# aleju/cat-generator

Measured on AMD Instinct MI355X. Metric: images/sec per G+D step, G32up-c 32x32 RGB bs=128 per GPU, higher is better.
Workload: dtype f32

## Files before the change

### cat-generator_amd/csrc/gemm.hip

```cpp
#include "common.h"
#include <stdlib.h>
#include <algorithm>
#include <mutex>
#include <type_traits>
#include <unordered_map>
#include <vector>

namespace {

typedef float f32x16 __attribute__((ext_vector_type(16)));
typedef unsigned int u32x4 __attribute__((ext_vector_type(4)));

constexpr int BK = 16;
constexpr unsigned OOB = 0x80000000u;
#ifdef CG_TRACE
__device__ unsigned long long* g_trace;
#define CG_STAMP(slot)                                                                                                  \
    do {                                                                                                                \
        if (threadIdx.x == 0 && g_trace) {                                                                              \
            const long wg = blockIdx.x + (long)gridDim.x * (blockIdx.y + (long)gridDim.y * blockIdx.z);                  \
            g_trace[wg * 8 + (slot)] = wall_clock64();                                                                  \
            if ((slot) == 0) {                                                                                          \
                g_trace[wg * 8 + 4] = __builtin_amdgcn_s_getreg((31 << 11) | 4);                       \
                g_trace[wg * 8 + 5] = __builtin_amdgcn_s_getreg((31 << 11) | 20);                     \
// ... 1614 lines not shown
    const int c = blockIdx.x * 32 + cl;
    float s = 0.f;
    if (c < Cout)
        for (int i = ln; i < S * P; i += 8) s += bp[(long)(i / P) * sstride + (long)(i % P) * Cout + c];
    sh[ln][cl] = s;
    __syncthreads();
    if (ln == 0 && c < Cout) {
        float t = 0.f;
#pragma unroll
        for (int r = 0; r < 8; ++r) t += sh[r][cl];
        gb[c] += scale * t;
    }
}

__global__ __launch_bounds__(256) void pack_weight_kernel(const float* w, float* wf, float* wb, int Cout, int Cin, int KK,
                                                          int wb_map) {
    __shared__ float sh[32][33];
    const int lo = threadIdx.x & 31, hi = threadIdx.x >> 5;
    const int ci0 = blockIdx.x * 32, co0 = blockIdx.y * 32;
    {
        const int tap = blockIdx.z;
#pragma unroll
        for (int j = 0; j < 4; ++j) {
            const int ci = ci0 + lo, co_l = hi + 8 * j, co = co0 + co_l;
            float v = 0.f;
            if (ci < Cin && co < Cout) {
                v = w[((long)co * Cin + ci) * KK + tap];
                if (wb) wb[wb_map ? ((long)co * KK + tap) * Cin + ci : ((long)(KK - 1 - tap) * Cout + co) * Cin + ci] = v;
            }
            sh[lo][co_l] = v;
        }
        if (wf) {
            __syncthreads();
#pragma unroll
            for (int j = 0; j < 4; ++j) {
                const int co = co0 + lo, ci_l = hi + 8 * j, ci = ci0 + ci_l;
                if (ci < Cin && co < Cout) wf[((long)tap * Cin + ci) * Cout + co] = sh[ci_l][lo];
            }
        }
    }
}

constexpr int kPackBatch = 48;
struct PackBatch {
    const float* w[kPackBatch]; float* wf[kPackBatch]; float* wb[kPackBatch];
    int Cout[kPackBatch], Cin[kPackBatch], KK[kPackBatch], first[kPackBatch + 1];
    unsigned long long map_mask;
    int n;
};
__global__ __launch_bounds__(256) void pack_weight_batch_kernel(PackBatch b) {
    __shared__ float sh[32][33];
    int e = 0;
    while (e + 1 < b.n && (int)blockIdx.x >= b.first[e + 1]) ++e;
    const float* w = b.w[e]; float* wf = b.wf[e]; float* wb = b.wb[e];
    const int Cout = b.Cout[e], Cin = b.Cin[e], KK = b.KK[e];
    const bool wb_map = (b.map_mask >> e) & 1ull;
    const int nbx = (Cin + 31) / 32, nby = (Cout + 31) / 32;
    int r = (int)blockIdx.x - b.first[e];
    const int bx = r % nbx; r /= nbx;
    const int by = r % nby;
    const int tap = r / nby;
    const int lo = threadIdx.x & 31, hi = threadIdx.x >> 5;
    const int ci0 = bx * 32, co0 = by * 32;
#pragma unroll
    for (int j = 0; j < 4; ++j) {
        const int ci = ci0 + lo, co_l = hi + 8 * j, co = co0 + co_l;
        float v = 0.f;
        if (ci < Cin && co < Cout) {
            v = w[((long)co * Cin + ci) * KK + tap];
            if (wb) wb[wb_map ? ((long)co * KK + tap) * Cin + ci : ((long)(KK - 1 - tap) * Cout + co) * Cin + ci] = v;
        }
        sh[lo][co_l] = v;
    }
    if (wf) {
        __syncthreads();
#pragma unroll
        for (int j = 0; j < 4; ++j) {
            const int co = co0 + lo, ci_l = hi + 8 * j, ci = ci0 + ci_l;
            if (ci < Cin && co < Cout) wf[((long)tap * Cin + ci) * Cout + co] = sh[ci_l][lo];
        }
    }
}

template <int K>
__global__ __launch_bounds__(256) void pack_weight_ups2_fast_kernel(const float* w, float* wf, float* wb, int Cout, int Cin) {
    constexpr int KK = K * K, PAD = (K - 1) / 2, KPD = K == 3 ? 2 : 3, KP = KPD * KPD;
    __shared__ float sh[KP][32][33];
    const int lo = threadIdx.x & 31, hi = threadIdx.x >> 5;
    const int ci0 = blockIdx.x * 32, co0 = blockIdx.y * 32;
    float v[4][KK];
#pragma unroll
    for (int j = 0; j < 4; ++j) {
        const int ci = ci0 + lo, co = co0 + hi + 8 * j;
        const bool ok = ci < Cin && co < Cout;
        const float* src = w + ((long)co * Cin + ci) * KK;
#pragma unroll
        for (int t = 0; t < KK; ++t) v[j][t] = ok ? src[t] : 0.f;
    }
#pragma unroll
    for (int p = 0; p < 4; ++p) {
#pragma unroll
        for (int j = 0; j < 4; ++j) {
            float acc[KP];
#pragma unroll
            for (int t = 0; t < KP; ++t) acc[t] = 0.f;
#pragma unroll
            for (int dy = 0; dy < K; ++dy)
#pragma unroll
                for (int dx = 0; dx < K; ++dx)
                    acc[phase_map(p >> 1, dy, PAD) * KPD + phase_map(p & 1, dx, PAD)] += v[j][dy * K + dx];
            const int ci = ci0 + lo, co_l = hi + 8 * j, co = co0 + co_l;
#pragma unroll
            for (int t = 0; t < KP; ++t) {
                if (wb && ci < Cin && co < Cout) wb[(((long)p * KP + t) * Cout + co) * Cin + ci] = acc[t];
                sh[t][lo][co_l] = acc[t];
            }
        }
        if (wf) {
            __syncthreads();
#pragma unroll
            for (int t = 0; t < KP; ++t)
#pragma unroll
                for (int j = 0; j < 4; ++j) {
                    const int co = co0 + lo, ci_l = hi + 8 * j, ci = ci0 + ci_l;
                    if (ci < Cin && co < Cout) wf[(((long)p * KP + t) * Cin + ci) * Cout + co] = sh[t][ci_l][lo];
                }
            __syncthreads();
        }
    }
}

__global__ __launch_bounds__(256) void pack_weight_ups2_kernel(const float* w, float* wf, float* wb, int Cout, int Cin, int k,
                                                               int pad, int kp, int CI_T) {
    extern __shared__ float sh[];
    const int KK = k * k, KP = kp * kp;
    const int run = CI_T * KK, ld = run + 1;
    const int ci0 = blockIdx.x * CI_T, co0 = blockIdx.y * 32;
    const int cis = min(CI_T, Cin - ci0);
    for (int idx = threadIdx.x; idx < 32 * run; idx += 256) {
        const int j = idx % run, co_l = idx / run;
        if (co0 + co_l < Cout && j < cis * KK) sh[co_l * ld + j] = w[((long)(co0 + co_l) * Cin + ci0) * KK + j];
    }
    __syncthreads();
    const int n = 4 * KP * CI_T * 32;
    for (int pass = 0; pass < 2; ++pass) {
        if (pass == 0 ? wf == nullptr : wb == nullptr) continue;
        for (int idx = threadIdx.x; idx < n; idx += 256) {
            int co_l, ci_l, q;
            if (pass == 0) { co_l = idx & 31; const int r = idx >> 5; ci_l = r % CI_T; q = r / CI_T; }
            else { ci_l = idx % CI_T; const int r = idx / CI_T; co_l = r & 31; q = r >> 5; }
            if (co0 + co_l >= Cout || ci_l >= cis) continue;
            const int tp = q % KP, p = q / KP;
            const int ry = tp / kp, rx = tp - ry * kp;
            const float* src = sh + co_l * ld + ci_l * KK;
            float s = 0.f;
            for (int dy = 0; dy < k; ++dy) {
                if (phase_map(p >> 1, dy, pad) != ry) continue;
                for (int dx = 0; dx < k; ++dx)
                    if (phase_map(p & 1, dx, pad) == rx) s += src[dy * k + dx];
            }
            if (pass == 0) wf[(((long)p * KP + tp) * Cin + ci0 + ci_l) * Cout + co0 + co_l] = s;
            else wb[(((long)p * KP + tp) * Cout + co0 + co_l) * Cin + ci0 + ci_l] = s;
        }
    }
}

template <int CO, int LP>
__global__ __launch_bounds__(256) void skinny_conv3x3_kernel(const float* __restrict__ x, const float* __restrict__ w,
                                                             const float* __restrict__ bias, float* __restrict__ y, int N,
                                                             int H, int W) {
    constexpr int Cin = 4 * LP;
    const int sub = threadIdx.x & (LP - 1);
    float wr[9][4][CO];
#pragma unroll
    for (int t = 0; t < 9; ++t)
#pragma unroll
        for (int j = 0; j < 4; ++j)
#pragma unroll
            for (int co = 0; co < CO; ++co) wr[t][j][co] = w[((long)t * Cin + sub * 4 + j) * CO + co];
    const long npix = (long)N * H * W;
    const long grp0 = (blockIdx.x * 256L + threadIdx.x) / LP;
    const long ngrp = gridDim.x * 256L / LP;
    const long iters = (npix + ngrp - 1) / ngrp;
    for (long it = 0; it < iters; ++it) {
        const long pix = grp0 + it * ngrp;
        const bool live = pix < npix;
        const unsigned pc = live ? (unsigned)pix : 0u;
        const unsigned row = pc / (unsigned)W;
        const int ox = (int)(pc - row * (unsigned)W), oy = (int)(row % (unsigned)H);
        const long n = row / (unsigned)H;
        float acc[CO];
#pragma unroll
        for (int co = 0; co < CO; ++co) acc[co] = 0.f;
        float4 v[9];
#pragma unroll
        for (int t = 0; t < 9; ++t) {
            const int iy = oy + t / 3 - 1, ix = ox + t % 3 - 1;
            const bool ok = live && iy >= 0 && iy < H && ix >= 0 && ix < W;
            const int cy = min(max(iy, 0), H - 1), cx = min(max(ix, 0), W - 1);
            const float4 q = ld4(x + ((n * H + cy) * (long)W + cx) * Cin + sub * 4);
            v[t] = ok ? q : make_float4(0.f, 0.f, 0.f, 0.f);
        }
#pragma unroll
        for (int t = 0; t < 9; ++t)
#pragma unroll
            for (int co = 0; co < CO; ++co)
                acc[co] += v[t].x * wr[t][0][co] + v[t].y * wr[t][1][co] + v[t].z * wr[t][2][co] + v[t].w * wr[t][3][co];
#pragma unroll
        for (int off = LP >> 1; off > 0; off >>= 1)
#pragma unroll
// ... 820 lines not shown
        CG_LAUNCH_CHECK();
        if (gb && gb[gi]) {
            hipLaunchKernelGGL(bias_part_reduce_kernel, dim3(cg::cdiv(Cout, 32)), dim3(256), 0, st,
                               (const float*)a.bias_part + (long)gi * g.nphase * Cout, gb[gi], p.splits, g.nphase,
                               (long)ZP * Cout, Cout, scale);
            CG_LAUNCH_CHECK();
        }
    }
    return 0;
}

}

int cg_conv2d_wgrad(void* stream, const float* x, const float* dy, float* gw, float* gb, int N, int Hp, int Wp, int Cin,
                    int Cout, int kH, int kW, int padH, int padW, int ups, float scale, void* ws, size_t ws_bytes) {
    CG_REQUIRE(x && dy && gw, "cg_conv2d_wgrad: null pointer");
    return cg_conv2d_wgrad_grouped(stream, 1, &x, &dy, &gw, &gb, N, Hp, Wp, Cin, Cout, kH, kW, padH, padW, ups, scale, ws,
                                   ws_bytes);
}

static int pack_ci_tile(int Cin, int KK) {
    int t = 1;
    while (t * 2 * KK <= 448 && t < Cin) t *= 2;
    return t;
}

int cg_pack_conv_weight(void* stream, const float* w, float* wf, float* wb, int Cout, int Cin, int kH, int kW) {
    CG_REQUIRE(w && (wf || wb), "cg_pack_conv_weight: null pointer");
    CG_REQUIRE(Cout > 0 && Cin > 0 && kH > 0 && kW > 0, "cg_pack_conv_weight: bad dims");
    const int KK = kH * kW;
    hipLaunchKernelGGL(pack_weight_kernel, dim3(cg::cdiv(Cin, 32), cg::cdiv(Cout, 32), KK), dim3(256), 0, cg::S(stream), w,
                       wf, wb, Cout, Cin, KK, 0);
    CG_LAUNCH_CHECK();
    return cg::wino3_note_pack(cg::S(stream), 1, &w, &wf, &wb, &Cout, &Cin, &kH, &kW, nullptr);
}

int cg_pack_conv_weight_map(void* stream, const float* w, float* wf, float* wbT, int Cout, int Cin, int kH, int kW) {
    CG_REQUIRE(w && (wf || wbT), "cg_pack_conv_weight_map: null pointer");
    CG_REQUIRE(Cout > 0 && Cin > 0 && kH > 0 && kW > 0, "cg_pack_conv_weight_map: bad dims");
    const int KK = kH * kW;
    hipLaunchKernelGGL(pack_weight_kernel, dim3(cg::cdiv(Cin, 32), cg::cdiv(Cout, 32), KK), dim3(256), 0, cg::S(stream), w,
                       wf, wbT, Cout, Cin, KK, 1);
    CG_LAUNCH_CHECK();
    return 0;
}

int cg_pack_conv_weight_batch(void* stream, int n, const float* const* w_canonical, float* const* wf, float* const* wb,
                              const int* Cout, const int* Cin, const int* kH, const int* kW, const int* wb_map) {
    CG_REQUIRE(n >= 0 && w_canonical && wf && wb && Cout && Cin && kH && kW, "cg_pack_conv_weight_batch: null pointer");
    for (int i0 = 0; i0 < n; i0 += kPackBatch) {
        PackBatch b;
        memset(&b, 0, sizeof(b));
        b.n = std::min(kPackBatch, n - i0);
        int blocks = 0;
        for (int e = 0; e < b.n; ++e) {
            const int i = i0 + e;
            CG_REQUIRE(w_canonical[i] && (wf[i] || wb[i]) && Cout[i] > 0 && Cin[i] > 0 && kH[i] > 0 && kW[i] > 0,
                       "cg_pack_conv_weight_batch: bad layer %d", i);
            b.w[e] = w_canonical[i]; b.wf[e] = wf[i]; b.wb[e] = wb[i];
            b.Cout[e] = Cout[i]; b.Cin[e] = Cin[i]; b.KK[e] = kH[i] * kW[i];
            if (wb_map && wb_map[i]) b.map_mask |= 1ull << e;
            b.first[e] = blocks;
            blocks += cg::cdiv(Cin[i], 32) * cg::cdiv(Cout[i], 32) * b.KK[e];
        }
        b.first[b.n] = blocks;
        hipLaunchKernelGGL(pack_weight_batch_kernel, dim3(blocks), dim3(256), 0, cg::S(stream), b);
        CG_LAUNCH_CHECK();
    }
    return cg::wino3_note_pack(cg::S(stream), n, w_canonical, wf, wb, Cout, Cin, kH, kW, wb_map);
}

size_t cg_pack_conv_weight_ups2_floats(int Cout, int Cin, int k, int pad) {
    if (Cout <= 0 || Cin <= 0 || k <= 0 || (k & 1) == 0 || pad != (k - 1) / 2) return 0;
    const int kp = phase_kp(k, pad);
    return (size_t)4 * kp * kp * Cin * Cout;
}

int cg_pack_conv_weight_ups2(void* stream, const float* w, float* wf_ph, float* wb_ph, int Cout, int Cin, int k, int pad) {
    CG_REQUIRE(w && (wf_ph || wb_ph), "cg_pack_conv_weight_ups2: null pointer");
    CG_REQUIRE(Cout > 0 && Cin > 0 && k > 0 && (k & 1) == 1 && pad == (k - 1) / 2,
               "cg_pack_conv_weight_ups2: needs an odd kernel with pad=(k-1)/2");
    const int kp = phase_kp(k, pad);
    CG_REQUIRE(k * k <= 448, "cg_pack_conv_weight_ups2: kernel too large (%d taps)", k * k);
    const dim3 fgrid(cg::cdiv(Cin, 32), cg::cdiv(Cout, 32));
    if (k == 3 || k == 5) {
        if (k == 3)
            hipLaunchKernelGGL(pack_weight_ups2_fast_kernel<3>, fgrid, dim3(256), 0, cg::S(stream), w, wf_ph, wb_ph, Cout, Cin);
        else
            hipLaunchKernelGGL(pack_weight_ups2_fast_kernel<5>, fgrid, dim3(256), 0, cg::S(stream), w, wf_ph, wb_ph, Cout, Cin);
        CG_LAUNCH_CHECK();
        return 0;
    }
    const int ci_t = pack_ci_tile(Cin, k * k);
    hipLaunchKernelGGL(pack_weight_ups2_kernel, dim3(cg::cdiv(Cin, ci_t), cg::cdiv(Cout, 32)), dim3(256),
                       (size_t)32 * (ci_t * k * k + 1) * sizeof(float), cg::S(stream), w, wf_ph, wb_ph, Cout, Cin, k, pad, kp,
                       ci_t);
    CG_LAUNCH_CHECK();
    return 0;
}

}

void cg::wgrad_discard_all() {
    std::lock_guard<std::mutex> lk(g_red_mu);
    for (auto& kv : g_red_queue) kv.second.clear();
}
```

### cat-generator_amd/csrc/winograd.hip

```cpp
#include "common.h"
#include <algorithm>
#include <type_traits>
#include <stdlib.h>

namespace {

typedef float f32x16 __attribute__((ext_vector_type(16)));

__device__ __forceinline__ float4 ld4(const float* p) { return *reinterpret_cast<const float4*>(p); }
__device__ __forceinline__ float wf4c(const float4& v, int i) { return i == 0 ? v.x : (i == 1 ? v.y : (i == 2 ? v.z : v.w)); }
__device__ __forceinline__ float4 f4add(float4 a, float4 b) { return make_float4(a.x + b.x, a.y + b.y, a.z + b.z, a.w + b.w); }
__device__ __forceinline__ float4 f4sub(float4 a, float4 b) { return make_float4(a.x - b.x, a.y - b.y, a.z - b.z, a.w - b.w); }

template <int MODE>
__global__ __launch_bounds__(256) void wino_input_transform_kernel(const float* __restrict__ src, float* __restrict__ V,
                                                                   int N, int Hl, int Wl, int C, int Cs) {
    const int cq_n = C >> 2;
    const int tH = Hl >> 1, tW = Wl >> 1;
    const long T = (long)N * tH * tW;
    const long total = T * cq_n;
    for (long idx = blockIdx.x * 256L + threadIdx.x; idx < total; idx += gridDim.x * 256L) {
        const int cq = (int)(idx % cq_n);
        const long tile = idx / cq_n;
        const int tj = (int)(tile % tW);
        const int ti = (int)((tile / tW) % tH);
        const long n = tile / ((long)tW * tH);
        int pa = 0, pb = 0, cs = cq * 4;
        if (MODE == 1) {
            const int p = cs / Cs;
            cs -= p * Cs;
            pa = p >> 1; pb = p & 1;
        }
        float4 d[4][4];
#pragma unroll
        for (int r = 0; r < 4; ++r)
#pragma unroll
            for (int c = 0; c < 4; ++c) {
                const int iy = 2 * ti - 1 + r, ix = 2 * tj - 1 + c;
                const bool ok = iy >= 0 && iy < Hl && ix >= 0 && ix < Wl;
                const int cy = min(max(iy, 0), Hl - 1), cx = min(max(ix, 0), Wl - 1);
                const float* ptr = MODE == 0 ? src + ((n * Hl + cy) * (long)Wl + cx) * C + cs
                                             : src + ((n * 2 * Hl + 2 * cy + pa) * (long)(2 * Wl) + 2 * cx + pb) * Cs + cs;
                const float4 q = ld4(ptr);
                d[r][c] = ok ? q : make_float4(0.f, 0.f, 0.f, 0.f);
            }
        float4 t[4][4];
#pragma unroll
        for (int c = 0; c < 4; ++c) {
            t[0][c] = f4sub(d[0][c], d[2][c]);
            t[1][c] = f4add(d[1][c], d[2][c]);
            t[2][c] = f4sub(d[2][c], d[1][c]);
            t[3][c] = f4sub(d[1][c], d[3][c]);
        }
        float* out = V + tile * C + cq * 4;
        const long xs = T * C;
#pragma unroll
        for (int r = 0; r < 4; ++r) {
            *reinterpret_cast<float4*>(out + (r * 4 + 0) * xs) = f4sub(t[r][0], t[r][2]);
            *reinterpret_cast<float4*>(out + (r * 4 + 1) * xs) = f4add(t[r][1], t[r][2]);
            *reinterpret_cast<float4*>(out + (r * 4 + 2) * xs) = f4sub(t[r][2], t[r][1]);
            *reinterpret_cast<float4*>(out + (r * 4 + 3) * xs) = f4sub(t[r][1], t[r][3]);
        }
    }
}

template <bool BWD>
__global__ __launch_bounds__(256) void wino_filter_transform_kernel(const float* __restrict__ src, float* __restrict__ U,
                                                                    int rows, int cols) {
    const int cqn = cols >> 2;
    const long plane = (long)rows * cols;
    const long total = 4L * rows * cqn;
    for (long idx = blockIdx.x * 256L + threadIdx.x; idx < total; idx += gridDim.x * 256L) {
        const int cq = (int)(idx % cqn);
        const int row = (int)((idx / cqn) % rows);
        const int p = (int)(idx / ((long)cqn * rows));
        float4 g[3][3];
#pragma unroll
        for (int ry = 0; ry < 3; ++ry)
#pragma unroll
            for (int rx = 0; rx < 3; ++rx) {
                const int tp = BWD ? (2 - ry) * 3 + (2 - rx) : ry * 3 + rx;
                g[ry][rx] = ld4(src + ((long)p * 9 + tp) * plane + (long)row * cols + cq * 4);
            }
        float4 t[4][3];
#pragma unroll
        for (int rx = 0; rx < 3; ++rx) {
            const float4 s = f4add(g[0][rx], g[2][rx]);
            t[0][rx] = g[0][rx];
            t[1][rx] = make_float4(0.5f * (s.x + g[1][rx].x), 0.5f * (s.y + g[1][rx].y), 0.5f * (s.z + g[1][rx].z), 0.5f * (s.w + g[1][rx].w));
            t[2][rx] = make_float4(0.5f * (s.x - g[1][rx].x), 0.5f * (s.y - g[1][rx].y), 0.5f * (s.z - g[1][rx].z), 0.5f * (s.w - g[1][rx].w));
            t[3][rx] = g[2][rx];
        }
#pragma unroll
        for (int xy = 0; xy < 4; ++xy) {
            const float4 s = f4add(t[xy][0], t[xy][2]);
            float4 o[4];
            o[0] = t[xy][0];
            o[1] = make_float4(0.5f * (s.x + t[xy][1].x), 0.5f * (s.y + t[xy][1].y), 0.5f * (s.z + t[xy][1].z), 0.5f * (s.w + t[xy][1].w));
            o[2] = make_float4(0.5f * (s.x - t[xy][1].x), 0.5f * (s.y - t[xy][1].y), 0.5f * (s.z - t[xy][1].z), 0.5f * (s.w - t[xy][1].w));
            o[3] = t[xy][2];
#pragma unroll
            for (int xx = 0; xx < 4; ++xx) {
                const int xi = xy * 4 + xx;
                float* dst = BWD ? U + ((long)xi * 4 * rows + (long)p * rows + row) * cols + cq * 4
                                 : U + (((long)p * 16 + xi) * rows + row) * cols + cq * 4;
                *reinterpret_cast<float4*>(dst) = o[xx];
            }
        }
    }
}

__global__ __launch_bounds__(256) void wino22_input_transform_kernel(const float* __restrict__ src, float* __restrict__ V, int N, int Hl,
                                                                     int Wl, int C) {
    const int cq_n = C >> 2;
    const int tH = Hl >> 1, tW = Wl >> 1;
    const long T = (long)N * tH * tW;
    const long total = T * cq_n;
    for (long idx = blockIdx.x * 256L + threadIdx.x; idx < total; idx += gridDim.x * 256L) {
        const int cq = (int)(idx % cq_n);
        const long tile = idx / cq_n;
        const int tj = (int)(tile % tW);
        const int ti = (int)((tile / tW) % tH);
        const long n = tile / ((long)tW * tH);
        float4 d[4][4];
#pragma unroll
        for (int r = 0; r < 4; ++r)
#pragma unroll
            for (int c = 0; c < 4; ++c) {
                const int iy = 2 * ti - 1 + r, ix = 2 * tj - 1 + c;
                const bool ok = iy >= 0 && iy < Hl && ix >= 0 && ix < Wl;
                const int cy = min(max(iy, 0), Hl - 1), cx = min(max(ix, 0), Wl - 1);
                const float4 q = ld4(src + ((n * Hl + cy) * (long)Wl + cx) * C + cq * 4);
                d[r][c] = ok ? q : make_float4(0.f, 0.f, 0.f, 0.f);
            }
        float* out = V + tile * C + cq * 4;
        const long xs = T * C;
#pragma unroll
        for (int a = 0; a < 2; ++a) {
            float4 t[3][4];
#pragma unroll
            for (int c = 0; c < 4; ++c) {
                t[0][c] = f4sub(d[a][c], d[a + 1][c]);
                t[1][c] = d[a + 1][c];
                t[2][c] = f4sub(d[a + 2][c], d[a + 1][c]);
            }
#pragma unroll
            for (int b = 0; b < 2; ++b) {
                const long pbase = (long)(a * 2 + b) * 9;
#pragma unroll
                for (int i = 0; i < 3; ++i) {
                    *reinterpret_cast<float4*>(out + (pbase + i * 3 + 0) * xs) = f4sub(t[i][b], t[i][b + 1]);
                    *reinterpret_cast<float4*>(out + (pbase + i * 3 + 1) * xs) = t[i][b + 1];
                    *reinterpret_cast<float4*>(out + (pbase + i * 3 + 2) * xs) = f4sub(t[i][b + 2], t[i][b + 1]);
                }
            }
        }
    }
}

__global__ __launch_bounds__(256) void wino22_dy_input_transform_kernel(const float* __restrict__ dy, float* __restrict__ V, int N, int Hl,
                                                                        int Wl, int Cs) {
    const int C = 4 * Cs, cq_n = C >> 2;
    const int tH = Hl >> 1, tW = Wl >> 1;
    const long T = (long)N * tH * tW;
    const long total = T * cq_n;
    for (long idx = blockIdx.x * 256L + threadIdx.x; idx < total; idx += gridDim.x * 256L) {
        const int cq = (int)(idx % cq_n);
        const long tile = idx / cq_n;
        const int tj = (int)(tile % tW);
        const int ti = (int)((tile / tW) % tH);
        const long n = tile / ((long)tW * tH);
        const int p = (cq * 4) / Cs, cs = cq * 4 - p * Cs;
        const int pa = p >> 1, pb = p & 1;
        float4 d[3][3];
#pragma unroll
        for (int r = 0; r < 3; ++r)
#pragma unroll
            for (int c = 0; c < 3; ++c) {
                const int iy = 2 * ti - pa + r, ix = 2 * tj - pb + c;
                const bool ok = iy >= 0 && iy < Hl && ix >= 0 && ix < Wl;
                const int cy = min(max(iy, 0), Hl - 1), cx = min(max(ix, 0), Wl - 1);
                const float4 q = ld4(dy + ((n * 2 * Hl + 2 * cy + pa) * (long)(2 * Wl) + 2 * cx + pb) * Cs + cs);
                d[r][c] = ok ? q : make_float4(0.f, 0.f, 0.f, 0.f);
            }
        float4 t[3][3];
#pragma unroll
        for (int c = 0; c < 3; ++c) { t[0][c] = f4sub(d[0][c], d[1][c]); t[1][c] = d[1][c]; t[2][c] = f4sub(d[2][c], d[1][c]); }
        float* out = V + tile * C + cq * 4;
        const long xs = T * C;
#pragma unroll
        for (int i = 0; i < 3; ++i) {
            *reinterpret_cast<float4*>(out + (i * 3 + 0) * xs) = f4sub(t[i][0], t[i][1]);
            *reinterpret_cast<float4*>(out + (i * 3 + 1) * xs) = t[i][1];
            *reinterpret_cast<float4*>(out + (i * 3 + 2) * xs) = f4sub(t[i][2], t[i][1]);
        }
    }
}

template <bool BWD>
__global__ __launch_bounds__(256) void wino22_filter_transform_kernel(const float* __restrict__ src, float* __restrict__ U, int rows,
                                                                      int cols) {
    const int cqn = cols >> 2;
    const long plane = (long)rows * cols;
    const long total = 4L * rows * cqn;
    for (long idx = blockIdx.x * 256L + threadIdx.x; idx < total; idx += gridDim.x * 256L) {
        const int cq = (int)(idx % cqn);
        const int row = (int)((idx / cqn) % rows);
        const int p = (int)(idx / ((long)cqn * rows));
        float4 g[2][2];
#pragma unroll
        for (int ry = 0; ry < 2; ++ry)
#pragma unroll
            for (int rx = 0; rx < 2; ++rx) {
                const int tp = BWD ? (1 - ry) * 2 + (1 - rx) : ry * 2 + rx;
                g[ry][rx] = ld4(src + ((long)p * 4 + tp) * plane + (long)row * cols + cq * 4);
            }
        float4 t[3][2];
#pragma unroll
        for (int rx = 0; rx < 2; ++rx) { t[0][rx] = g[0][rx]; t[1][rx] = f4add(g[0][rx], g[1][rx]); t[2][rx] = g[1][rx]; }
#pragma unroll
        for (int i = 0; i < 3; ++i) {
            float* dst = BWD ? U + ((long)(i * 3) * 4 * rows + (long)p * rows + row) * cols + cq * 4
                             : U + (((long)p * 9 + i * 3) * rows + row) * cols + cq * 4;
            const long xstep = BWD ? 4 * plane : plane;
            *reinterpret_cast<float4*>(dst) = t[i][0];
            *reinterpret_cast<float4*>(dst + xstep) = f4add(t[i][0], t[i][1]);
            *reinterpret_cast<float4*>(dst + 2 * xstep) = t[i][1];
        }
    }
}

struct WinoArgs {
    const float* V;
    const float* U;
    const float* bias;
    float* y;
    int T, K, Nc;
    int tH, tW;
    int so;
    int Ho, Wo;
    float* stats;
    int xcd;
    int vpp;
    int kz;
    int lg_tw, lg_th;
};

template <int NW, int BK>
__global__ __launch_bounds__(64 * NW, 4) void wino_gemm_kernel(WinoArgs a) {
    static_assert(NW == 8, "8 waves per workgroup");
    constexpr int BM = 64, BN = 128, NI = 8 / NW, NT = 64 * NW;
    constexpr int KV = BK / 4;
    constexpr int BQ = BK * 32 / NT;
    static_assert(BM * KV <= NT && (BQ == 1 || BQ == 2), "staging layout");
    constexpr int A_TILE = BK * BM, B_TILE = BK * BN;
    __shared__ __attribute__((aligned(16))) float smem[2 * A_TILE + 2 * B_TILE];
    float* As = smem;
    float* Bs = smem + 2 * A_TILE;
    const int tid = threadIdx.x, lane = tid & 63, wave = tid >> 6;
    const int l31 = lane & 31, h = lane >> 5;
    const int wm0 = (wave & 1) * 32, wn0 = (wave >> 1) * (32 * NI);
    const int ntn = a.Nc / BN;
    int tn = blockIdx.x % ntn, tm = blockIdx.x / ntn, phase = blockIdx.z;
    const int tiles_m = gridDim.x / ntn;
    if (a.xcd && (tiles_m & 7) == 0) {
        const int share = ntn * (int)gridDim.z;
        const int L = (int)blockIdx.z * (int)gridDim.x + (int)blockIdx.x;
        const int slot = L >> 3, member = slot % share;
        tm = (slot / share) * 8 + (L & 7);
        phase = member / ntn;
        tn = member - phase * ntn;
    }
    const int m0 = tm * BM, n0 = tn * BN;
    const int KT = CG_PROBE_HALF(4, a.K / BK);

    const int a_kv = tid % KV, a_r = (tid / KV) % BM;
    const bool a_thr = tid < BM * KV;
    const int a_row = min(m0 + a_r, a.T - 1);
    const int b_kr = tid >> 5, b_nv = tid & 31;
    const float* Ap = a.V + (long)a_row * a.K + 4 * a_kv;
    const float* Bp = a.U + (long)phase * 16 * a.K * a.Nc + (long)b_kr * a.Nc + n0 + 4 * b_nv;
    const long a_xi = (long)a.T * a.K;
    const long b_half = (long)(NT / 32) * a.Nc;
    float4 areg, breg0, breg1;
    const float* Ac = Ap;
    const float* Bc = Bp;
    const long b_step = (long)BK * a.Nc;
    const long a_jump = a_xi - a.K + BK;
    auto load_next = [&](bool last_kt) {
        Ac += last_kt ? a_jump : (long)BK;
        Bc += b_step;
        if (BM * KV == NT || a_thr) areg = ld4(Ac);
        breg0 = ld4(Bc);
        if (BQ == 2) breg1 = ld4(Bc + b_half);
    };
    const int a_so = a_r ^ (BK == 32 ? ((a_kv & 7) << 2) : ((a_kv & 3) << 3));
    auto store_tile = [&](int buf) {
        float* A = As + buf * A_TILE;
        float* B = Bs + buf * B_TILE;
        if (BM * KV == NT || a_thr) {
            A[(4 * a_kv + 0) * BM + a_so] = areg.x;
            A[(4 * a_kv + 1) * BM + a_so] = areg.y;
            A[(4 * a_kv + 2) * BM + a_so] = areg.z;
            A[(4 * a_kv + 3) * BM + a_so] = areg.w;
        }
        *reinterpret_cast<float4*>(B + b_kr * BN + 4 * b_nv) = breg0;
        if (BQ == 2) *reinterpret_cast<float4*>(B + (b_kr + NT / 32) * BN + 4 * b_nv) = breg1;
    };

    f32x16 accM[NI], accY[4][NI];
#pragma unroll
    for (int j = 0; j < NI; ++j)
// ... 322 lines not shown
    double a = 0.0;
    if (co < Cout)
        for (int b = rl; b < nblocks; b += 8) {
            const float* row = bpart + (long)b * 4 * Cout + co;
            a += ((double)row[0] + (double)row[Cout]) + ((double)row[2 * Cout] + (double)row[3 * Cout]);
        }
    sh[rl][cl] = a;
    __syncthreads();
    if (rl == 0 && co < Cout) {
        double t = 0.0;
#pragma unroll
        for (int r = 0; r < 8; ++r) t += sh[r][cl];
        gb[co] += scale * (float)t;
    }
}

__device__ __host__ __forceinline__ int wino_phase_map(int a, int d) { return ((a + d - 2) >> 1) - ((a - 2) >> 1); }

__global__ __launch_bounds__(256) void wino_wgrad_finish_kernel(const float* __restrict__ dUt, float* __restrict__ gw, int Cout,
                                                                int Cin, float scale) {
    const long total = (long)Cout * Cin;
    const long xs = 4L * Cout * Cin;
    for (long idx = blockIdx.x * 256L + threadIdx.x; idx < total; idx += gridDim.x * 256L) {
        const int ci = (int)(idx % Cin);
        const int co = (int)(idx / Cin);
        float acc[25];
#pragma unroll
        for (int t = 0; t < 25; ++t) acc[t] = 0.f;
#pragma unroll
        for (int p = 0; p < 4; ++p) {
            float u[4][4];
#pragma unroll
            for (int xi = 0; xi < 16; ++xi) u[xi >> 2][xi & 3] = dUt[xi * xs + ((long)p * Cout + co) * Cin + ci];
            float t[3][4];
#pragma unroll
            for (int c = 0; c < 4; ++c) {
                t[0][c] = u[0][c] + 0.5f * (u[1][c] + u[2][c]);
                t[1][c] = 0.5f * (u[1][c] - u[2][c]);
                t[2][c] = 0.5f * (u[1][c] + u[2][c]) + u[3][c];
            }
            float g[3][3];
#pragma unroll
            for (int r = 0; r < 3; ++r) {
                g[r][0] = t[r][0] + 0.5f * (t[r][1] + t[r][2]);
                g[r][1] = 0.5f * (t[r][1] - t[r][2]);
                g[r][2] = 0.5f * (t[r][1] + t[r][2]) + t[r][3];
            }
#pragma unroll
            for (int dy = 0; dy < 5; ++dy)
#pragma unroll
                for (int dx = 0; dx < 5; ++dx) acc[dy * 5 + dx] += g[wino_phase_map(p >> 1, dy)][wino_phase_map(p & 1, dx)];
        }
        float* dst = gw + idx * 25;
#pragma unroll
        for (int t = 0; t < 25; ++t) dst[t] += scale * acc[t];
    }
}


__device__ __host__ __forceinline__ int wino22_phase_map(int a, int d) { return ((a + d - 1) >> 1) - ((a - 1) >> 1); }


static bool wino_dims_ok(int N, int Hp, int Wp, int Cin, int Cout) {
    return N > 0 && Hp > 0 && Wp > 0 && (Hp & 1) == 0 && (Wp & 1) == 0 && Cin > 0 && Cout > 0 && Cin % 128 == 0 &&
           Cout % 128 == 0  && (long)N * Hp * Wp * std::max(Cin, 4 * Cout) * 4L < (1L << 40);
}

}

extern "C" {

size_t cg_conv2d_ups2_wino_supported(int N, int Hp, int Wp, int Cin, int Cout, int k, int pad) {
    return k == 5 && pad == 2 && wino_dims_ok(N, Hp, Wp, Cin, Cout) ? 1 : 0;
}
size_t cg_conv2d_ups2_wino_v_floats(int N, int Hp, int Wp, int C) {
    return (size_t)16 * ((size_t)N * (Hp / 2) * (Wp / 2)) * C;
}
size_t cg_conv2d_ups2_wino_u_floats(int Cin, int Cout) { return (size_t)4 * 16 * Cin * Cout; }

int cg_conv2d_ups2_wino_pack(void* stream, const float* wf_ph, const float* wb_ph, float* u_fwd, float* u_bwd, int Cout,
                             int Cin) {
    CG_REQUIRE((wf_ph && u_fwd) || (wb_ph && u_bwd), "cg_conv2d_ups2_wino_pack: null pointer");
    CG_REQUIRE(Cin % 4 == 0 && Cout % 4 == 0, "cg_conv2d_ups2_wino_pack: channel counts must be multiples of 4");
    if (wf_ph && u_fwd) {
        const long total = 4L * Cin * (Cout / 4);
        hipLaunchKernelGGL(wino_filter_transform_kernel<false>, dim3(cg::ew_grid(total)), dim3(256), 0, cg::S(stream), wf_ph,
                           u_fwd, Cin, Cout);
        CG_LAUNCH_CHECK();
    }
    if (wb_ph && u_bwd) {
        const long total = 4L * Cout * (Cin / 4);
        hipLaunchKernelGGL(wino_filter_transform_kernel<true>, dim3(cg::ew_grid(total)), dim3(256), 0, cg::S(stream), wb_ph,
                           u_bwd, Cout, Cin);
        CG_LAUNCH_CHECK();
    }
    return 0;
}

static int wino_gemm_launch(void* stream, const float* v, const float* u, const float* bias, float* y, int N, int Hp, int Wp,
                            int Cin, int Cout, int dgrad, float* stats, int npos = 16, int kslices = 1);

int cg_conv2d_ups2_wino_gemm(void* stream, const float* v, const float* u, const float* bias, float* y, int N, int Hp, int Wp,
                             int Cin, int Cout, int dgrad) {
    return wino_gemm_launch(stream, v, u, bias, y, N, Hp, Wp, Cin, Cout, dgrad, nullptr);
}

size_t cg_conv2d_ups2_wino_stats_rows(int N, int Hp, int Wp, int Cin, int Cout) {
    if (!wino_dims_ok(N, Hp, Wp, Cin, Cout)) return 0;
    return (size_t)4 * cg::cdiv((long)N * (Hp / 2) * (Wp / 2), 64) * 2;
}

static int wino_gemm_launch(void* stream, const float* v, const float* u, const float* bias, float* y, int N, int Hp, int Wp,
                            int Cin, int Cout, int dgrad, float* stats, int npos, int kslices) {
    CG_REQUIRE(v && u && y, "cg_conv2d_ups2_wino_gemm: null pointer");
    CG_REQUIRE(wino_dims_ok(N, Hp, Wp, Cin, Cout), "cg_conv2d_ups2_wino_gemm: unsupported dimensions");
    const int T = N * (Hp / 2) * (Wp / 2);
    WinoArgs a;
    a.V = v; a.U = u; a.bias = bias; a.y = y; a.T = T; a.tH = Hp / 2; a.tW = Wp / 2; a.stats = stats;
    a.xcd = (int)cg::opt(cg::OPT_XCD_SWIZZLE);
    a.vpp = npos == 9 && !dgrad ? 1 : 0;
    a.kz = 0;
    a.lg_tw = a.lg_th = -1;
    CG_REQUIRE(!stats || !dgrad, "wino_gemm: statistics only on the forward launch");
    if (dgrad) { a.K = 4 * Cout; a.Nc = Cin; a.so = 1; a.Ho = Hp; a.Wo = Wp; }
    else { a.K = Cin; a.Nc = Cout; a.so = 2; a.Ho = 2 * Hp; a.Wo = 2 * Wp; }
    const int bk = (int)cg::opt(cg::OPT_WINO_BK);
    CG_REQUIRE(kslices <= 1 || (dgrad && a.K % kslices == 0 && (a.K / kslices) % 64 == 0), "wino_gemm: K slices only on the data gradient, in multiples of 64 rows");
    if (kslices > 1) a.kz = a.K / kslices;
    {
        auto lg = [](int v) { int l = 0; while ((1 << l) < v) ++l; return (1 << l) == v ? l : -1; };
        const long ybytes = (long)N * a.Ho * a.Wo * a.Nc * 4L;
        if (lg(a.tW) >= 0 && lg(a.tH) >= 0 && ybytes < 0x7fffffffL) { a.lg_tw = lg(a.tW); a.lg_th = lg(a.tH); }
    }
    const dim3 grid(cg::cdiv(T, 64) * (a.Nc / 128), 1, dgrad ? (kslices > 1 ? kslices : 1) : 4);
    const bool k32 = bk == 32 || (bk == 0 && (long)grid.x * grid.z <= cg::kNumCU * 3 / 2);
    const bool glds = cg::opt(cg::OPT_WINO_GLDS) != 0 && (long)T * a.K * 4L < 0x7fffffffL &&
                      16L * a.K * a.Nc * 4L < 0x7fffffffL;
    if (npos == 9) {
        CG_REQUIRE(glds, "wino_gemm: the 9-position form needs the LDS-direct-load kernel (CG_WINO_GLDS)");
        if (k32 && (a.kz ? a.kz : a.K) % 64 == 0) hipLaunchKernelGGL((wino_gemm_g_kernel<32, 9>), grid, dim3(512), 0, cg::S(stream), a);
        else hipLaunchKernelGGL((wino_gemm_g_kernel<16, 9>), grid, dim3(512), 0, cg::S(stream), a);
        CG_LAUNCH_CHECK();
        return 0;
    }
    CG_REQUIRE(kslices <= 1 || glds, "wino_gemm: K slices need the LDS-direct-load kernel (CG_WINO_GLDS)");
    if (glds && k32 && (a.kz ? a.kz : a.K) % 64 == 0) { hipLaunchKernelGGL((wino_gemm_g_kernel<32>), grid, dim3(512), 0, cg::S(stream), a); CG_LAUNCH_CHECK(); return 0; }
    if (glds) { hipLaunchKernelGGL((wino_gemm_g_kernel<16>), grid, dim3(512), 0, cg::S(stream), a); CG_LAUNCH_CHECK(); return 0; }
    if (k32 && a.K % 64 == 0) hipLaunchKernelGGL((wino_gemm_kernel<8, 32>), grid, dim3(512), 0, cg::S(stream), a);
    else hipLaunchKernelGGL((wino_gemm_kernel<8, 16>), grid, dim3(512), 0, cg::S(stream), a);
    CG_LAUNCH_CHECK();
    return 0;
}

int cg_conv2d_ups2_wino_forward_stats(void* stream, const float* x_lo, const float* u_fwd, const float* bias, float* y, float* v,
                                      int N, int Hp, int Wp, int Cin, int Cout, float* stats) {
    CG_REQUIRE(x_lo && u_fwd && y && v, "cg_conv2d_ups2_wino_forward: null pointer");
    CG_REQUIRE(wino_dims_ok(N, Hp, Wp, Cin, Cout), "cg_conv2d_ups2_wino_forward: unsupported dimensions");
    hipStream_t st = cg::S(stream);
    const int T = N * (Hp / 2) * (Wp / 2);
    hipLaunchKernelGGL(wino_input_transform_kernel<0>, dim3(cg::ew_grid((long)T * (Cin / 4))), dim3(256), 0, st, x_lo, v, N, Hp,
                       Wp, Cin, Cin);
    CG_LAUNCH_CHECK();
    return wino_gemm_launch(stream, v, u_fwd, bias, y, N, Hp, Wp, Cin, Cout, 0, stats);
}

int cg_conv2d_ups2_wino_forward(void* stream, const float* x_lo, const float* u_fwd, const float* bias, float* y, float* v,
                                int N, int Hp, int Wp, int Cin, int Cout) {
    return cg_conv2d_ups2_wino_forward_stats(stream, x_lo, u_fwd, bias, y, v, N, Hp, Wp, Cin, Cout, nullptr);
}

size_t cg_conv2d_ups2_wino22_supported(int N, int Hp, int Wp, int Cin, int Cout) {
    if (!wino_dims_ok(N, Hp, Wp, Cin, Cout)) return 0;
    const long T = (long)N * (Hp / 2) * (Wp / 2);
    const bool glds = cg::opt(cg::OPT_WINO_GLDS) != 0 && T * Cin * 4L < 0x7fffffffL &&
                      16L * Cin * Cout * 4L < 0x7fffffffL;
    return glds ? 1 : 0;
}
size_t cg_conv2d_ups2_wino22_dgrad_supported(int N, int Hp, int Wp, int Cin, int Cout) {
    return cg_conv2d_ups2_wino22_supported(N, Hp, Wp, Cin, Cout) && (long)N * (Hp / 2) * (Wp / 2) * Cout * 16L < 0x7fffffffL ? 1 : 0;
}
size_t cg_conv2d_ups2_wino22_v_floats(int N, int Hp, int Wp, int Cin) { return (size_t)36 * ((size_t)N * (Hp / 2) * (Wp / 2)) * Cin; }
size_t cg_conv2d_ups2_wino22_u_floats(int Cin, int Cout) { return (size_t)4 * 9 * Cin * Cout; }

int cg_conv2d_ups2_wino22_pack(void* stream, const float* wf_ph, const float* wb_ph, float* u_fwd, float* u_bwd, int Cout, int Cin) {
    CG_REQUIRE((wf_ph && u_fwd) || (wb_ph && u_bwd), "cg_conv2d_ups2_wino22_pack: null pointer");
    CG_REQUIRE(Cin % 4 == 0 && Cout % 4 == 0, "cg_conv2d_ups2_wino22_pack: channel counts must be multiples of 4");
    if (wf_ph && u_fwd) {
        hipLaunchKernelGGL(wino22_filter_transform_kernel<false>, dim3(cg::ew_grid(4L * Cin * (Cout / 4))), dim3(256), 0, cg::S(stream), wf_ph,
                           u_fwd, Cin, Cout);
        CG_LAUNCH_CHECK();
    }
    if (wb_ph && u_bwd) {
        hipLaunchKernelGGL(wino22_filter_transform_kernel<true>, dim3(cg::ew_grid(4L * Cout * (Cin / 4))), dim3(256), 0, cg::S(stream), wb_ph,
                           u_bwd, Cout, Cin);
        CG_LAUNCH_CHECK();
    }
    return 0;
}

int cg_conv2d_ups2_wino22_forward_stats(void* stream, const float* x_lo, const float* u22, const float* bias, float* y, float* v,
                                        int N, int Hp, int Wp, int Cin, int Cout, float* stats) {
    CG_REQUIRE(x_lo && u22 && y && v, "cg_conv2d_ups2_wino22_forward: null pointer");
    CG_REQUIRE(cg_conv2d_ups2_wino22_supported(N, Hp, Wp, Cin, Cout), "cg_conv2d_ups2_wino22_forward: unsupported dimensions / options");
    const int T = N * (Hp / 2) * (Wp / 2);
    hipLaunchKernelGGL(wino22_input_transform_kernel, dim3(cg::ew_grid((long)T * (Cin / 4))), dim3(256), 0, cg::S(stream), x_lo, v, N, Hp, Wp, Cin);
    CG_LAUNCH_CHECK();
    return wino_gemm_launch(stream, v, u22, bias, y, N, Hp, Wp, Cin, Cout, 0, stats, 9);
}

static int wino22_dgrad_slices(int N, int Hp, int Wp, int Cin, int Cout) {
    if (Cout % 64 != 0) return 1;
    return (long)cg::cdiv(N * (Hp / 2) * (Wp / 2), 64) * (Cin / 128) < cg::kNumCU ? 4 : 1;
}

extern "C++" template <int S>
__global__ __launch_bounds__(256) void wino22_sum_kernel(const float* __restrict__ part, float* __restrict__ out, long n4, long stride) {
    for (long i = blockIdx.x * 256L + threadIdx.x; i < n4; i += gridDim.x * 256L) {
        const float4 a = ld4(part + 4 * i), b = ld4(part + stride + 4 * i);
        float4 r = f4add(a, b);
        if (S == 4) r = f4add(r, f4add(ld4(part + 2 * stride + 4 * i), ld4(part + 3 * stride + 4 * i)));
        *reinterpret_cast<float4*>(out + 4 * i) = r;
    }
}

size_t cg_conv2d_ups2_wino22_dgrad_v_floats(int N, int Hp, int Wp, int Cin, int Cout) {
    const size_t T = (size_t)N * (Hp / 2) * (Wp / 2);
    const int sl = wino22_dgrad_slices(N, Hp, Wp, Cin, Cout);
    return 36 * T * Cout + (sl > 1 ? (size_t)sl * 4 * T * Cin : 0);
}

int cg_conv2d_ups2_wino22_dgrad(void* stream, const float* dy, const float* u_bwd, float* dx_lo, float* v_dy, int N, int Hp, int Wp, int Cin,
                                int Cout) {
    CG_REQUIRE(dy && u_bwd && dx_lo && v_dy, "cg_conv2d_ups2_wino22_dgrad: null pointer");
    CG_REQUIRE(cg_conv2d_ups2_wino22_dgrad_supported(N, Hp, Wp, Cin, Cout), "cg_conv2d_ups2_wino22_dgrad: unsupported dimensions / options");
    const int T = N * (Hp / 2) * (Wp / 2);
    hipLaunchKernelGGL(wino22_dy_input_transform_kernel, dim3(cg::ew_grid((long)T * Cout)), dim3(256), 0, cg::S(stream), dy, v_dy, N, Hp, Wp, Cout);
    CG_LAUNCH_CHECK();
    const int sl = wino22_dgrad_slices(N, Hp, Wp, Cin, Cout);
    if (sl == 1) return wino_gemm_launch(stream, v_dy, u_bwd, nullptr, dx_lo, N, Hp, Wp, Cin, Cout, 1, nullptr, 9);
    float* part = v_dy + (size_t)36 * T * Cout;
    if (wino_gemm_launch(stream, v_dy, u_bwd, nullptr, part, N, Hp, Wp, Cin, Cout, 1, nullptr, 9, sl)) return 1;
    const long n = (long)T * 4 * Cin;
    if (sl == 4) hipLaunchKernelGGL(wino22_sum_kernel<4>, dim3(cg::ew_grid(n / 4)), dim3(256), 0, cg::S(stream), part, dx_lo, n / 4, n);
    else hipLaunchKernelGGL(wino22_sum_kernel<2>, dim3(cg::ew_grid(n / 4)), dim3(256), 0, cg::S(stream), part, dx_lo, n / 4, n);
    CG_LAUNCH_CHECK();
    return 0;
}

int cg_conv2d_ups2_wino_dgrad(void* stream, const float* dy, const float* u_bwd, float* dx_lo, float* v_dy, int N, int Hp,
                              int Wp, int Cin, int Cout) {
    CG_REQUIRE(dy && u_bwd && dx_lo && v_dy, "cg_conv2d_ups2_wino_dgrad: null pointer");
    CG_REQUIRE(wino_dims_ok(N, Hp, Wp, Cin, Cout), "cg_conv2d_ups2_wino_dgrad: unsupported dimensions");
    hipStream_t st = cg::S(stream);
    const int T = N * (Hp / 2) * (Wp / 2);
    hipLaunchKernelGGL(wino_input_transform_kernel<1>, dim3(cg::ew_grid((long)T * Cout)), dim3(256), 0, st, dy, v_dy, N, Hp, Wp,
                       4 * Cout, Cout);
    CG_LAUNCH_CHECK();
    return cg_conv2d_ups2_wino_gemm(stream, v_dy, u_bwd, nullptr, dx_lo, N, Hp, Wp, Cin, Cout, 1);
}

static int wino_dgrad_slices(int N, int Hp, int Wp, int Cin, int Cout) {
    const int force = 0;
    const long T = (long)N * (Hp / 2) * (Wp / 2);
    const bool glds = cg::opt(cg::OPT_WINO_GLDS) != 0 && T * 4L * Cout * 4L < 0x7fffffffL &&
                      16L * 4L * Cout * Cin * 4L < 0x7fffffffL;
    if (!glds || !wino_dims_ok(N, Hp, Wp, Cin, Cout)) return 1;
    const long wgs = (long)cg::cdiv((int)T, 64) * (Cin / 128);
    int sl = force == 1 || force == 2 || force == 4 ? force : (wgs >= cg::kNumCU ? 1 : (wgs * 2 >= cg::kNumCU ? 2 : 4));
    while (sl > 1 && (4 * Cout / sl) % 64 != 0) sl >>= 1;
    return sl;
}
size_t cg_conv2d_ups2_wino_dgrad_part_floats(int N, int Hp, int Wp, int Cin, int Cout) {
    const int sl = wino_dgrad_slices(N, Hp, Wp, Cin, Cout);
    return sl > 1 ? (size_t)sl * N * Hp * Wp * Cin : 0;
}
int cg_conv2d_ups2_wino_dgrad_split(void* stream, const float* dy, const float* u_bwd, float* dx_lo, float* v_dy, float* part, int N, int Hp,
                                    int Wp, int Cin, int Cout) {
    const int sl = wino_dgrad_slices(N, Hp, Wp, Cin, Cout);
    if (sl <= 1 || !part) return cg_conv2d_ups2_wino_dgrad(stream, dy, u_bwd, dx_lo, v_dy, N, Hp, Wp, Cin, Cout);
// ... 66 lines not shown
```

Measured before the change: 22860.

## Restructure ups2 weight pack per phase and merge fwd/bwd winograd filter transforms

The ups2 phase weight-pack kernel now uses 16x16 channel tiles with one phase per grid z-slice. Each tile is staged into shared memory with coalesced loads, and the fwd and bwd layouts are computed from shared memory in two passes. This replaces the old 32x32 tile with per-phase transposes and barriers, raising parallelism and cutting register pressure. Separately, the forward and backward winograd filter transforms (both variants) are merged into one launch that splits blocks by index, saving a kernel launch per weight pack.

```diff
diff --git a/cat-generator_amd/csrc/gemm.hip b/cat-generator_amd/csrc/gemm.hip
--- a/cat-generator_amd/csrc/gemm.hip
+++ b/cat-generator_amd/csrc/gemm.hip
@@ -1720,50 +1720,49 @@
     }
 }
 
+constexpr int kPackUpsT = 16;
+template <int K, int P>
+__device__ __forceinline__ void pack_ups2_phase_sums(const float* src, float* acc) {
+    constexpr int PAD = (K - 1) / 2, KPD = K == 3 ? 2 : 3, KP = KPD * KPD;
+#pragma unroll
+    for (int t = 0; t < KP; ++t) acc[t] = 0.f;
+#pragma unroll
+    for (int dy = 0; dy < K; ++dy)
+#pragma unroll
+        for (int dx = 0; dx < K; ++dx) acc[phase_map(P >> 1, dy, PAD) * KPD + phase_map(P & 1, dx, PAD)] += src[dy * K + dx];
+}
 template <int K>
-__global__ __launch_bounds__(256) void pack_weight_ups2_fast_kernel(const float* w, float* wf, float* wb, int Cout, int Cin) {
-    constexpr int KK = K * K, PAD = (K - 1) / 2, KPD = K == 3 ? 2 : 3, KP = KPD * KPD;
-    __shared__ float sh[KP][32][33];
-    const int lo = threadIdx.x & 31, hi = threadIdx.x >> 5;
-    const int ci0 = blockIdx.x * 32, co0 = blockIdx.y * 32;
-    float v[4][KK];
-#pragma unroll
-    for (int j = 0; j < 4; ++j) {
-        const int ci = ci0 + lo, co = co0 + hi + 8 * j;
-        const bool ok = ci < Cin && co < Cout;
-        const float* src = w + ((long)co * Cin + ci) * KK;
-#pragma unroll
-        for (int t = 0; t < KK; ++t) v[j][t] = ok ? src[t] : 0.f;
-    }
-#pragma unroll
-    for (int p = 0; p < 4; ++p) {
-#pragma unroll
-        for (int j = 0; j < 4; ++j) {
-            float acc[KP];
-#pragma unroll
-            for (int t = 0; t < KP; ++t) acc[t] = 0.f;
-#pragma unroll
-            for (int dy = 0; dy < K; ++dy)
-#pragma unroll
-                for (int dx = 0; dx < K; ++dx)
-                    acc[phase_map(p >> 1, dy, PAD) * KPD + phase_map(p & 1, dx, PAD)] += v[j][dy * K + dx];
-            const int ci = ci0 + lo, co_l = hi + 8 * j, co = co0 + co_l;
-#pragma unroll
-            for (int t = 0; t < KP; ++t) {
-                if (wb && ci < Cin && co < Cout) wb[(((long)p * KP + t) * Cout + co) * Cin + ci] = acc[t];
-                sh[t][lo][co_l] = acc[t];
-            }
-        }
-        if (wf) {
-            __syncthreads();
-#pragma unroll
-            for (int t = 0; t < KP; ++t)
-#pragma unroll
-                for (int j = 0; j < 4; ++j) {
-                    const int co = co0 + lo, ci_l = hi + 8 * j, ci = ci0 + ci_l;
-                    if (ci < Cin && co < Cout) wf[(((long)p * KP + t) * Cin + ci) * Cout + co] = sh[t][ci_l][lo];
-                }
-            __syncthreads();
+__global__ __launch_bounds__(256) void pack_weight_ups2_fast_kernel(const float* __restrict__ w, float* __restrict__ wf,
+                                                                    float* __restrict__ wb, int Cout, int Cin) {
+    constexpr int T = kPackUpsT, KK = K * K, KPD = K == 3 ? 2 : 3, KP = KPD * KPD, RUN = T * KK, LD = RUN + 1;
+    __shared__ float sh[T * LD];
+    const int ci0 = blockIdx.x * T, co0 = blockIdx.y * T, p = blockIdx.z;
+    const int cis = min(T, Cin - ci0), cos = min(T, Cout - co0);
+    for (int idx = threadIdx.x; idx < T * RUN; idx += 256) {
+        const int co_l = idx / RUN, j = idx - co_l * RUN;
+        if (co_l < cos && j < cis * KK) sh[co_l * LD + j] = w[((long)(co0 + co_l) * Cin + ci0) * KK + j];
+    }
+    __syncthreads();
+    const int lo = threadIdx.x & (T - 1), hi = threadIdx.x >> 4;
+#pragma unroll
+    for (int pass = 0; pass < 2; ++pass) {
+        float* dst = pass == 0 ? wb : wf;
+        const int ci_l = pass == 0 ? lo : hi, co_l = pass == 0 ? hi : lo;
+        if (!dst || ci_l >= cis || co_l >= cos) continue;
+        const float* src = sh + co_l * LD + ci_l * KK;
+        float acc[KP];
+        switch (p) {
+            case 0: pack_ups2_phase_sums<K, 0>(src, acc); break;
+            case 1: pack_ups2_phase_sums<K, 1>(src, acc); break;
+            case 2: pack_ups2_phase_sums<K, 2>(src, acc); break;
+            default: pack_ups2_phase_sums<K, 3>(src, acc); break;
+        }
+        const long ci = ci0 + ci_l, co = co0 + co_l;
+#pragma unroll
+        for (int t = 0; t < KP; ++t) {
+            const long q = (long)p * KP + t;
+            if (pass == 0) wb[(q * Cout + co) * Cin + ci] = acc[t];
+            else wf[(q * Cin + ci) * Cout + co] = acc[t];
         }
     }
 }
@@ -2750,8 +2749,9 @@
                "cg_pack_conv_weight_ups2: needs an odd kernel with pad=(k-1)/2");
     const int kp = phase_kp(k, pad);
     CG_REQUIRE(k * k <= 448, "cg_pack_conv_weight_ups2: kernel too large (%d taps)", k * k);
-    const dim3 fgrid(cg::cdiv(Cin, 32), cg::cdiv(Cout, 32));
+    const dim3 fgrid(cg::cdiv(Cin, kPackUpsT), cg::cdiv(Cout, kPackUpsT), 4);
     if (k == 3 || k == 5) {
+        CG_REQUIRE(fgrid.y <= 65535u, "cg_pack_conv_weight_ups2: too many output planes (%d)", Cout);
         if (k == 3)
             hipLaunchKernelGGL(pack_weight_ups2_fast_kernel<3>, fgrid, dim3(256), 0, cg::S(stream), w, wf_ph, wb_ph, Cout, Cin);
         else
diff --git a/cat-generator_amd/csrc/winograd.hip b/cat-generator_amd/csrc/winograd.hip
--- a/cat-generator_amd/csrc/winograd.hip
+++ b/cat-generator_amd/csrc/winograd.hip
@@ -65,12 +65,12 @@
 }
 
 template <bool BWD>
-__global__ __launch_bounds__(256) void wino_filter_transform_kernel(const float* __restrict__ src, float* __restrict__ U,
-                                                                    int rows, int cols) {
+__device__ __forceinline__ void wino_filter_transform(const float* __restrict__ src, float* __restrict__ U, int rows, int cols,
+                                                      long block, long nblocks) {
     const int cqn = cols >> 2;
     const long plane = (long)rows * cols;
     const long total = 4L * rows * cqn;
-    for (long idx = blockIdx.x * 256L + threadIdx.x; idx < total; idx += gridDim.x * 256L) {
+    for (long idx = block * 256L + threadIdx.x; idx < total; idx += nblocks * 256L) {
         const int cq = (int)(idx % cqn);
         const int row = (int)((idx / cqn) % rows);
         const int p = (int)(idx / ((long)cqn * rows));
@@ -108,6 +108,13 @@
             }
         }
     }
+}
+__global__ __launch_bounds__(256) void wino_filter_transform_kernel(const float* __restrict__ wf_ph, const float* __restrict__ wb_ph,
+                                                                    float* __restrict__ u_fwd, float* __restrict__ u_bwd, int Cout,
+                                                                    int Cin, int nblk_f) {
+    const int b = (int)blockIdx.x;
+    if (b < nblk_f) wino_filter_transform<false>(wf_ph, u_fwd, Cin, Cout, b, nblk_f);
+    else wino_filter_transform<true>(wb_ph, u_bwd, Cout, Cin, b - nblk_f, (long)gridDim.x - nblk_f);
 }
 
 __global__ __launch_bounds__(256) void wino22_input_transform_kernel(const float* __restrict__ src, float* __restrict__ V, int N, int Hl,
@@ -198,12 +205,12 @@
 }
 
 template <bool BWD>
-__global__ __launch_bounds__(256) void wino22_filter_transform_kernel(const float* __restrict__ src, float* __restrict__ U, int rows,
-                                                                      int cols) {
+__device__ __forceinline__ void wino22_filter_transform(const float* __restrict__ src, float* __restrict__ U, int rows, int cols,
+                                                        long block, long nblocks) {
     const int cqn = cols >> 2;
     const long plane = (long)rows * cols;
     const long total = 4L * rows * cqn;
-    for (long idx = blockIdx.x * 256L + threadIdx.x; idx < total; idx += gridDim.x * 256L) {
+    for (long idx = block * 256L + threadIdx.x; idx < total; idx += nblocks * 256L) {
         const int cq = (int)(idx % cqn);
         const int row = (int)((idx / cqn) % rows);
         const int p = (int)(idx / ((long)cqn * rows));
@@ -228,6 +235,13 @@
             *reinterpret_cast<float4*>(dst + 2 * xstep) = t[i][1];
         }
     }
+}
+__global__ __launch_bounds__(256) void wino22_filter_transform_kernel(const float* __restrict__ wf_ph, const float* __restrict__ wb_ph,
+                                                                      float* __restrict__ u_fwd, float* __restrict__ u_bwd, int Cout,
+                                                                      int Cin, int nblk_f) {
+    const int b = (int)blockIdx.x;
+    if (b < nblk_f) wino22_filter_transform<false>(wf_ph, u_fwd, Cin, Cout, b, nblk_f);
+    else wino22_filter_transform<true>(wb_ph, u_bwd, Cout, Cin, b - nblk_f, (long)gridDim.x - nblk_f);
 }
 
 struct WinoArgs {
@@ -716,18 +730,9 @@
                              int Cin) {
     CG_REQUIRE((wf_ph && u_fwd) || (wb_ph && u_bwd), "cg_conv2d_ups2_wino_pack: null pointer");
     CG_REQUIRE(Cin % 4 == 0 && Cout % 4 == 0, "cg_conv2d_ups2_wino_pack: channel counts must be multiples of 4");
-    if (wf_ph && u_fwd) {
-        const long total = 4L * Cin * (Cout / 4);
-        hipLaunchKernelGGL(wino_filter_transform_kernel<false>, dim3(cg::ew_grid(total)), dim3(256), 0, cg::S(stream), wf_ph,
-                           u_fwd, Cin, Cout);
-        CG_LAUNCH_CHECK();
-    }
-    if (wb_ph && u_bwd) {
-        const long total = 4L * Cout * (Cin / 4);
-        hipLaunchKernelGGL(wino_filter_transform_kernel<true>, dim3(cg::ew_grid(total)), dim3(256), 0, cg::S(stream), wb_ph,
-                           u_bwd, Cout, Cin);
-        CG_LAUNCH_CHECK();
-    }
+    const int nf = wf_ph && u_fwd ? cg::ew_grid(4L * Cin * (Cout / 4)) : 0, nb = wb_ph && u_bwd ? cg::ew_grid(4L * Cout * (Cin / 4)) : 0;
+    hipLaunchKernelGGL(wino_filter_transform_kernel, dim3(nf + nb), dim3(256), 0, cg::S(stream), wf_ph, wb_ph, u_fwd, u_bwd, Cout, Cin, nf);
+    CG_LAUNCH_CHECK();
     return 0;
 }
 
@@ -819,16 +824,9 @@
 int cg_conv2d_ups2_wino22_pack(void* stream, const float* wf_ph, const float* wb_ph, float* u_fwd, float* u_bwd, int Cout, int Cin) {
     CG_REQUIRE((wf_ph && u_fwd) || (wb_ph && u_bwd), "cg_conv2d_ups2_wino22_pack: null pointer");
     CG_REQUIRE(Cin % 4 == 0 && Cout % 4 == 0, "cg_conv2d_ups2_wino22_pack: channel counts must be multiples of 4");
-    if (wf_ph && u_fwd) {
-        hipLaunchKernelGGL(wino22_filter_transform_kernel<false>, dim3(cg::ew_grid(4L * Cin * (Cout / 4))), dim3(256), 0, cg::S(stream), wf_ph,
-                           u_fwd, Cin, Cout);
-        CG_LAUNCH_CHECK();
-    }
-    if (wb_ph && u_bwd) {
-        hipLaunchKernelGGL(wino22_filter_transform_kernel<true>, dim3(cg::ew_grid(4L * Cout * (Cin / 4))), dim3(256), 0, cg::S(stream), wb_ph,
-                           u_bwd, Cout, Cin);
-        CG_LAUNCH_CHECK();
-    }
+    const int nf = wf_ph && u_fwd ? cg::ew_grid(4L * Cin * (Cout / 4)) : 0, nb = wb_ph && u_bwd ? cg::ew_grid(4L * Cout * (Cin / 4)) : 0;
+    hipLaunchKernelGGL(wino22_filter_transform_kernel, dim3(nf + nb), dim3(256), 0, cg::S(stream), wf_ph, wb_ph, u_fwd, u_bwd, Cout, Cin, nf);
+    CG_LAUNCH_CHECK();
     return 0;
 }
 
```

Result: no change. 23070, median of 6 (+0.9%).
